# 10XGenomics/thermite

Measured on AMD Instinct MI355X. Metric: aligned reads/sec (91 bp), higher is better.
Workload: dtype i32

## Files before the change

thermite_amd/capi.py:

```python
import ctypes as C
import os

import numpy as np

from .refdata import EXON_DT, REF_DT, SPAN_DT, TX_DT

_HERE = os.path.dirname(os.path.abspath(__file__))
SO_PATH = os.environ.get("THM_LIB") or os.path.join(_HERE, "_build", "libthermite_amd.so")

MEM_DT = np.dtype([("ref_idx", "<u8"), ("query_idx", "<u4"), ("len", "<u4")])
ALN_DT = np.dtype(
    [
        ("ystart", "<u8"),
        ("yend", "<u8"),
        ("ylen", "<u8"),
        ("ops_off", "<u8"),
        ("tx_ystart", "<u8"),
        ("tx_yend", "<u8"),
        ("tx_ylen", "<u8"),
        ("tx_ops_off", "<u8"),
        ("score", "<i4"),
        ("ref_id", "<u4"),
        ("xstart", "<u4"),
        ("xend", "<u4"),
# ... 239 lines not shown
    L.thm_writer_header.restype = i32
    L.thm_writer_header.argtypes = [vp, vp]
    L.thm_writer_trailer.restype = i32
    L.thm_writer_trailer.argtypes = [vp, vp]
    L.thm_writer_format_batch.restype = i32
    L.thm_writer_format_batch.argtypes = [vp, vp, vp, vp]
    L.thm_writer_format_batch_cigars.restype = i32
    L.thm_writer_format_batch_cigars.argtypes = [vp, vp, vp, vp]
    L.thm_batch_upload_reads.restype = i32
    L.thm_batch_upload_reads.argtypes = [vp, vp]
    L.thm_batch_fetch_bam.restype = i32
    L.thm_batch_fetch_bam.argtypes = [vp, u32, vp]
    L.thm_align_batch_bam.restype = i32
    L.thm_align_batch_bam.argtypes = [vp, vp, u32, vp]
    L.thm_writer_wrap_bam.restype = i32
    L.thm_writer_wrap_bam.argtypes = [vp, vp, vp]
    L.thm_align_files.restype = i32
    L.thm_align_files.argtypes = [vp, vp, u32, cp, i32, u64, u32, vp]
    L.thm_align_files_multi.restype = i32
    L.thm_align_files_multi.argtypes = [vp, u32, vp, u32, cp, i32, u64, u32, vp]
    if hasattr(L, "thm_debug_prof_get"):
        L.thm_debug_prof_get.restype = i32
        L.thm_debug_prof_get.argtypes = [vp, vp, i32]
    if hasattr(L, "thm_debug_set_pool_caps"):
        L.thm_debug_set_pool_caps.restype = i32
        L.thm_debug_set_pool_caps.argtypes = [vp, u64, u64, u64, vp]
    if hasattr(L, "thm_debug_set_flags"):
        L.thm_debug_set_flags.restype = i32
        L.thm_debug_set_flags.argtypes = [vp, C.c_uint32]
        L.thm_debug_set_band_clip.restype = i32
        L.thm_debug_set_band_clip.argtypes = [vp, C.c_uint32]
        L.thm_debug_tpr_stats.restype = i32
        L.thm_debug_tpr_stats.argtypes = [vp, vp]
    if hasattr(L, "thm_debug_knobs"):
        L.thm_debug_knobs.restype = i32
        L.thm_debug_knobs.argtypes = [vp, vp]
    if hasattr(L, "thm_debug_calib_gather"):
        L.thm_debug_calib_gather.restype = i32
        L.thm_debug_calib_gather.argtypes = [vp, i32, u64, vp]
    if hasattr(L, "thm_debug_wave_prims"):
        L.thm_debug_wave_prims.restype = i32
        L.thm_debug_wave_prims.argtypes = [vp, vp, vp]
    _lib = L
    return L


def _ptr(a):
    return a.ctypes.data_as(C.c_void_p) if a is not None else None


def _copy(ptr, count, dtype, copy=True):
    if count == 0 or not ptr:
        return np.zeros(0, dtype=dtype)
    nbytes = int(count) * np.dtype(dtype).itemsize
    buf = (C.c_uint8 * nbytes).from_address(ptr)
    a = np.frombuffer(buf, dtype=dtype, count=int(count))
    return a.copy() if copy else a


def _u8(b):
    if isinstance(b, np.ndarray):
        return np.ascontiguousarray(b, np.uint8)
    return np.frombuffer(bytes(b), np.uint8)


def build_suffix_array_gpu(text, wide=False):
# ... 338 lines not shown
                                                  _ptr(hits), len(hits), _ptr(bw), _ptr(xd), max_band_width, C.byref(v)))
        status = (_copy(v.hit_status, v.n_hits, "<i4") if v.hit_status else np.zeros(int(v.n_hits), "<i4"))
        return _copy(v.alns, v.n_hits, ALN_DT), _copy(v.ops, v.n_op_bytes, np.uint8), status

    def counters(self):
        out = np.zeros(N_COUNTERS, "<u8")
        self._chk(lib().thm_counters_get(self.h, _ptr(out)))
        return out

    def reset_counters(self):
        self._chk(lib().thm_counters_reset(self.h))

    def counters_allreduce(self, comm):
        self._chk(lib().thm_counters_allreduce(self.h, comm.h))

    def counters_device_ptr(self):
        return lib().thm_counters_device_ptr(self.h)

    def timings(self):
        out = np.zeros(N_TIMINGS, "<f4")
        self._chk(lib().thm_timings_get(self.h, _ptr(out)))
        return dict(zip(TIMING_NAMES, out.tolist()))

    def debug_prof(self, reset=True):
        out = np.zeros(16, "<u8")
        self._chk(lib().thm_debug_prof_get(self.h, _ptr(out), int(reset)))
        return out

    def debug_set_pool_caps(self, smem_cap=0, cand_cap=0, ops_cap=0):
        n = C.c_uint32()
        self._chk(lib().thm_debug_set_pool_caps(self.h, smem_cap, cand_cap, ops_cap, C.byref(n)))
        return n.value

    def debug_set_flags(self, tpr=None, rounds=0):
        self._chk(lib().thm_debug_set_flags(self.h, (0 if tpr is None else (2 if tpr else 1)) | (int(rounds) << 8)))

    def debug_set_band_clip(self, max_bw=None):
        self._chk(lib().thm_debug_set_band_clip(self.h, 0 if max_bw is None else int(max_bw) + 1))

    def debug_tpr_stats(self):
        out = np.zeros(32, "<u8")
        self._chk(lib().thm_debug_tpr_stats(self.h, _ptr(out)))
        return out

    def debug_knobs(self):
        out = np.zeros(16, "<u4")
        self._chk(lib().thm_debug_knobs(self.h, _ptr(out)))
        return out

    def debug_calib_gather(self, pattern, n_threads):
        b = C.c_uint64()
        self._chk(lib().thm_debug_calib_gather(self.h, pattern, n_threads, C.byref(b)))
        return b.value

    def debug_wave_prims(self, v):
        v = np.ascontiguousarray(v, "<i4")
        out = np.zeros(384, "<i4")
        self._chk(lib().thm_debug_wave_prims(self.h, _ptr(v), _ptr(out)))
        return out.reshape(6, 64)

    def close(self):
        if getattr(self, "h", None):
            lib().thm_aligner_free(self.h)
            self.h = None

    def __del__(self):
        self.close()

# ... 183 lines not shown
```

thermite_amd/csrc/aligner.hip:

```cpp
#include <hip/hip_runtime.h>

#include <algorithm>
#include <cstdarg>
#include <cstdio>
#include <cstdlib>
#include <cstring>
#include <mutex>
#include <string>
#include <type_traits>
#include <vector>

#include "aligner_internal.h"

namespace thm {
const char* global_error_cstr();
}
using namespace thm;

static int swg_blocks_per_cu() {
  static const int v = [] {
    const char* e = getenv("THM_SWG_BPC");
    const int v = e ? atoi(e) : 4;
    return (v >= 1 && v <= 8) ? v : 4;
  }();
// ... 483 lines not shown
  out->n = n;
  out->n_op_bytes = a->h_ops.size();
  out->alns = a->h_lr.data();
  out->ops = a->h_ops.data();
  return THM_OK;
}

int32_t thm_debug_prof_get(thm_aligner* a, uint64_t out[16], int32_t reset) {
  if (!a || !out) return THM_ERR_INVALID_ARG;
  HIPCHK(a, hipSetDevice(a->device));
  uint8_t* p = a->d_counters.as<uint8_t>() + 2 * THM_N_COUNTERS * 8;
  HIPCHK(a, hipMemcpyAsync(out, p, 16 * 8, hipMemcpyDeviceToHost, a->stream));
  if (reset) HIPCHK(a, hipMemsetAsync(p, 0, 16 * 8, a->stream));
  HIPCHK(a, hipStreamSynchronize(a->stream));
  return THM_OK;
}

int32_t thm_debug_set_pool_caps(thm_aligner* a, uint64_t smem_cap, uint64_t cand_cap, uint64_t ops_cap, uint32_t* n_replays) {
  if (!a) return THM_ERR_INVALID_ARG;
  a->dbg_smem_cap = smem_cap;
  a->dbg_cand_cap = cand_cap;
  a->dbg_ops_cap = ops_cap;
  a->smem_cap = a->cand_cap = a->cand_ops_cap = 0;
  if (n_replays) *n_replays = a->n_replays;
  return THM_OK;
}

int32_t thm_debug_set_flags(thm_aligner* a, uint32_t flags) {
  if (!a) return THM_ERR_INVALID_ARG;
  if (flags & 1u) a->use_tpr = false;
  if (flags & 2u) a->use_tpr = true;
  const int r = (int)((flags >> 8) & 15u);
  if (r >= 1 && r <= TPR_MAX_ROUNDS) a->tpr_rounds = r;
  return THM_OK;
}
int32_t thm_debug_set_band_clip(thm_aligner* a, uint32_t max_bw_plus_1) {
  if (!a) return THM_ERR_INVALID_ARG;
  a->dbg_band_clip = max_bw_plus_1;
  return THM_OK;
}
int32_t thm_debug_tpr_stats(thm_aligner* a, uint64_t stats[32]) {
  if (!a || !stats) return THM_ERR_INVALID_ARG;
  memset(stats, 0, 256);
  if (!a->t_ctl.p) return THM_OK;
  HIPCHK(a, hipSetDevice(a->device));
  HIPCHK(a, hipStreamSynchronize(a->stream));
  unsigned long long c[40];
  HIPCHK(a, hipMemcpy(c, a->t_ctl.p, sizeof c, hipMemcpyDeviceToHost));
  for (int k = 0; k < 16; k++) stats[k] = c[TPRC_STATS + k];
  stats[16] = c[TPRC_REC_CUR];
  stats[17] = c[TPRC_Q_CUR];
  for (int k = 0; k < 4; k++) stats[18 + k] = c[TPRC_Q_CUR + 1 + k];
  stats[22] = c[TPRC_N_ACT + a->tpr_rounds + 1];
  return THM_OK;
}
int32_t thm_debug_knobs(thm_aligner* a, uint32_t out[16]) {
  if (!a || !out) return THM_ERR_INVALID_ARG;
  out[0] = seed_fill_mode();
  out[1] = (uint32_t)compact_k();
  out[2] = (uint32_t)hit_gl();
  for (int cpl = 1; cpl <= 4; cpl++)
    for (int wide = 0; wide < 2; wide++) out[3 + 2 * (cpl - 1) + wide] = (uint32_t)extend_waves_per_simd(cpl, wide != 0);
  out[11] = team_div_per_cu();
  out[12] = (uint32_t)swg_blocks_per_cu();
  out[13] = a->use_tpr ? 1u : 0u;
  out[14] = (uint32_t)a->tpr_rounds;
// ... 29 lines not shown
```

thermite_amd/csrc/aligner_internal.h:

```cpp
#ifndef THERMITE_ALIGNER_INTERNAL_H
#define THERMITE_ALIGNER_INTERNAL_H
#include <hip/hip_runtime.h>

#include <cstdarg>
#include <cstdio>
#include <string>
#include <vector>

#include "launch.h"
#include "thermite_internal.h"

struct DBuf {
  void* p = nullptr;
  size_t cap = 0;
  hipError_t ensure(size_t bytes) {
    if (bytes <= cap) return hipSuccess;
    if (p) (void)hipFree(p);
    p = nullptr;
    cap = 0;
    size_t want = bytes + bytes / 4 + 256;
    hipError_t e = hipMalloc(&p, want);
    if (e == hipSuccess) cap = want;
    return e;
  }
// ... 62 lines not shown
  hipStream_t stream3 = nullptr;
  hipEvent_t ev_join3 = nullptr;
  hipStream_t stream4 = nullptr;
  hipEvent_t ev_dpt_fork = nullptr, ev_dpt_join = nullptr;
  hipEvent_t ev_fork = nullptr, ev_join = nullptr;
  thm_align_opts opts;
  std::string err;

  DBuf d_counters, d_queue, d_fault, d_cursors;
  DBuf b0, b1, b2, b3, b4, b5, b6, b7, b8;

  DBuf r_bases, r_offsets, r_san;
  DBuf r_status;
  uint64_t n_reads = 0, n_bases = 0;
  uint32_t max_read_len = 0;
  std::vector<std::pair<uint32_t, uint64_t>> len_hist;
  uint64_t n_over = 0;
  bool uploaded = false;
  DBuf s_smems, s_off, s_cnt, s_hits, s_cand_off, scan_tmp, s_ms_end, s_ms_lo, s_ms_hi, s_work_reads, s_work_long, s_work_cells,
      s_work_counts, s_sel_scratch, s_heavy, s_slow, s_team, s_fill_keys, s_fill_perm, s_fill_hist;
  uint64_t smem_cap = 0;
  DBuf e_heavy, e_rel;
  DBuf e_cands, e_order, e_ops, e_nalns, e_nalns64, e_opbytes, e_aln_off, e_ops_off, e_trace, e_slow, e_recs, e_wcnt;
  DBuf t_memos, t_recs, t_dpops, t_qlist, t_act[2], t_ctl, t_bail, t_queue2, t_trace, t_ttrace, t_hdr, t_sums;
  bool use_tpr = false;
  int tpr_rounds = 8;
  uint64_t n_slow_host = 0;
  uint32_t fast_max_len = 0, slow_max_len = 0;
  uint64_t cand_cap = 0, cand_ops_cap = 0;
  DBuf o_alns, o_ops, o_mems;
  uint64_t out_alns_cap = 0, out_ops_cap = 0;
  uint64_t dbg_smem_cap = 0, dbg_cand_cap = 0, dbg_ops_cap = 0;
  uint32_t dbg_band_clip = 0;
  uint32_t n_replays = 0;
  bool ran = false, synced = false;
  hipEvent_t ev[6] = {nullptr, nullptr, nullptr, nullptr, nullptr, nullptr};
  float timings[THM_N_TIMINGS] = {0};

  HBuf r_off[2], r_alns[2], r_ops[2], r_stat[2];
  int r_cur = 0;
  std::vector<uint64_t> h_off;
  std::vector<thm_aln> h_alns;
  std::vector<uint8_t> h_ops;
  std::vector<thm_mem> h_mems;
  std::vector<thm_swg_aln> h_swg;
  std::vector<thm_lr_aln> h_lr;
  DBuf sh_bases, sh_san, sh_off, sh_hits, sh_read, sh_bw, sh_xd, sh_list, sh_out, sh_status, sh_ops, sh_ctl, sh_trace, sh_slow;
  std::vector<thm_aln> h_hit_alns;
  std::vector<int32_t> h_hit_status;
  std::vector<uint8_t> h_hit_ops;
  DBuf c_sums, c_nwords, c_woff, c_scan_tmp, c_flags, c_dig, c_words, c_in_ops, c_in_off;
  HBuf ch_off[2], ch_alns[2], ch_dig[2], ch_words[2], ch_stat[2];
  int c_cur = 0;
  hipEvent_t ev_cig[4] = {nullptr, nullptr, nullptr, nullptr};
  std::vector<thm_aln_digest> h_cig_dig;
  std::vector<uint32_t> h_cig_words;
  DBuf bn_names, bn_name_off, bn_quals;
  bool reads_named = false, reads_have_quals = false;
  DBuf bt_tx_pool, bt_tx_off, bt_gid_pool, bt_gid_off, bt_gname_pool, bt_gname_off, bt_tx_gene, bt_ref_sq;
  bool bam_tables = false;
  DBuf bm_cnt, bm_first, bm_qn, bm_rec_read, bm_len, bm_off, bm_out, bm_read_off, bm_err, bm_scan_tmp;
  HBuf bh_data[2], bh_off[2], bh_stat[2];
  int b_cur = 0;
  int bam_stage = -1;
  hipEvent_t ev_bam[4] = {nullptr, nullptr, nullptr, nullptr};
};
// ... 28 lines not shown
```

thermite_amd/csrc/kernels_seed.hip:

```cpp
#include <hip/hip_runtime.h>

#include <algorithm>

#include "launch.h"
#include "swg_device.h"

namespace thm {
namespace dev {

__device__ __forceinline__ int base_code(uint8_t c) {
  return c == 'A' ? 0 : c == 'C' ? 1 : c == 'G' ? 2 : c == 'T' ? 3 : -1;
}
__device__ __forceinline__ uint8_t sanitize_base(uint8_t c) {
  if (c >= 'a' && c <= 'z') c = (uint8_t)(c - 32);
  return (c == 'A' || c == 'C' || c == 'G' || c == 'T' || c == 'N') ? c : (uint8_t)0;
}
__device__ __forceinline__ uint64_t load8_global(const uint8_t* p) {
  uint64_t v;
  __builtin_memcpy(&v, p, 8);
  return v;
}
__device__ __forceinline__ uint64_t load8_lds(const uint8_t* base16, int off) {
  const uint64_t* q = (const uint64_t*)(base16 + (off & ~7));
  const unsigned sh = (unsigned)(off & 7) * 8u;
// ... 14 lines not shown
        *less = ((tw >> (8 * idx)) & 0xff) < ((qw >> (8 * idx)) & 0xff);
        return idx;
      }
      return cap;
    }
    o = 8;
  }
  while (o < cap) {
    uint64_t tw[8];
#pragma unroll
    for (int u = 0; u < 8; u++) tw[u] = load8_global(tp + o + 8 * u);
#pragma unroll
    for (int u = 0; u < 8; u++) {
      const int oo = o + 8 * u;
      if (oo < cap) {
        const uint64_t qw = load8_global(q + oo);
        const uint64_t x = tw[u] ^ qw;
        if (x) {
          const int idx = __builtin_ctzll(x) >> 3;
          if (oo + idx < cap) {
            *less = ((tw[u] >> (8 * idx)) & 0xff) < ((qw >> (8 * idx)) & 0xff);
            return oo + idx;
          }
          return cap;
        }
      }
    }
    o += 64;
  }
  return cap;
}

template <class C>
__device__ void ms_search(const DeviceIndexT<C>& ix, const uint8_t* rd, int L, int pos, int k, int& out_d, C& out_lo, C& out_hi) {
  C lo = 0, hi = (C)ix.n;
  int d = 0;
  const int kt = (int)ix.kt;
  if (kt <= k) {
    uint32_t code = 0;
    bool acgt = true;
    const uint64_t w0 = load8_global(rd + pos), w1 = load8_global(rd + pos + 8);
    for (int t = 0; t < kt; t++) {
      const int c = base_code((uint8_t)((t < 8 ? (w0 >> (8 * t)) : (w1 >> (8 * (t - 8)))) & 0xff));
      acgt = acgt && (c >= 0);
      code = (code << 2) | (uint32_t)(c & 3);
    }
    if (acgt) {
      const LutEntryT<C> e = ix.lut[code];
      lo = e.lo;
      hi = e.hi;
      d = kt;
    }
  }
  if (lo < hi && pos + d < L) {
    const int cap = L - (pos + d);
    const uint8_t* q = rd + pos + d;
    bool less;
    const C sz = hi - lo;
    if (sz == 1) {
      d += lcp_cmp<false>(ix.text + ix.sa[lo] + d, q, cap, &less);
    } else if (q[0] != 0) {
      if (sz <= 8) {
        C sav[8];
        uint64_t tw[8];
        int lc[8];
#pragma unroll
        for (int u = 0; u < 8; u++) sav[u] = (lo + u < hi) ? ix.sa[lo + u] : (C)0;
#pragma unroll
        for (int u = 0; u < 8; u++) tw[u] = load8_global(ix.text + sav[u] + d);
        const uint64_t qw = load8_global(q);
        int ms = 0;
#pragma unroll
        for (int u = 0; u < 8; u++) {
          const uint64_t x = tw[u] ^ qw;
          int l = x ? (__builtin_ctzll(x) >> 3) : 8;
          l = min(l, cap);
          if (lo + u >= hi) l = -1;
          lc[u] = l;
        }
#pragma unroll
        for (int u = 0; u < 8; u++) {
          if (lc[u] == 8 && cap > 8) lc[u] = 8 + lcp_cmp<false>(ix.text + sav[u] + d + 8, q + 8, cap - 8, &less);
          ms = max(ms, lc[u]);
        }
// ... 28 lines not shown
          C nlo = a, nhi = a;
          if (l1 >= ms) {
            C x = lo, y = a - 1;
            while (x < y) {
              const C m = x + ((y - x) >> 1);
              if (lcp_cmp<true>(ix.text + ix.sa[m] + d, q, ms, &less) >= ms)
                y = m;
              else
                x = m + 1;
            }
            nlo = x;
          }
          if (l2 >= ms) {
            C x = a + 1, y = hi;
            while (x < y) {
              const C m = x + ((y - x) >> 1);
              if (lcp_cmp<true>(ix.text + ix.sa[m] + d, q, ms, &less) >= ms)
                x = m + 1;
              else
                y = m;
            }
            nhi = x;
          }
          lo = nlo;
          hi = nhi;
          d += ms;
        }
      }
    }
  }
  out_d = (lo < hi) ? d : 0;
  out_lo = lo;
  out_hi = hi;
}

__global__ void sanitize_kernel(const uint8_t* in, uint8_t* out, uint64_t n, uint64_t n_padded) {
  const uint64_t i = ((uint64_t)blockIdx.x * blockDim.x + threadIdx.x) * 16;
  if (i >= n_padded) return;
  uint4 v = make_uint4(0, 0, 0, 0);
  if (i < n) v = *(const uint4*)(in + i);
  uint32_t w[4] = {v.x, v.y, v.z, v.w};
#pragma unroll
  for (int j = 0; j < 4; j++) {
    uint32_t r = 0;
#pragma unroll
    for (int b = 0; b < 4; b++) {
      const uint64_t at = i + (uint64_t)(4 * j + b);
      const uint8_t c = (at < n) ? sanitize_base((uint8_t)(w[j] >> (8 * b))) : (uint8_t)0;
      r |= (uint32_t)c << (8 * b);
    }
    w[j] = r;
  }
  *(uint4*)(out + i) = make_uint4(w[0], w[1], w[2], w[3]);
}

constexpr int PROBE_STRIDE = 8;

__device__ __forceinline__ void block_append(bool flag, unsigned long long value, unsigned long long* list,
                                             unsigned long long* count) {
  __shared__ unsigned w_cnt[4];
  __shared__ unsigned long long b_base;
  const unsigned long long m = __ballot(flag);
  const int lane = lane_id(), wv = (int)(threadIdx.x >> 6);
  if (lane == 0) w_cnt[wv] = (unsigned)__popcll(m);
  __syncthreads();
  if (threadIdx.x == 0) {
    const unsigned total = w_cnt[0] + w_cnt[1] + w_cnt[2] + w_cnt[3];
    b_base = total ? atomicAdd(count, (unsigned long long)total) : 0ull;
  }
  __syncthreads();
  unsigned before = 0;
  for (int w = 0; w < wv; w++) before += w_cnt[w];
  if (flag) list[b_base + before + (unsigned long long)__popcll(m & ((1ull << lane) - 1ull))] = value;
  __syncthreads();
}

template <class C>
__global__ __launch_bounds__(256) void seed_first_kernel(SeedParamsT<C> p) {
  const uint64_t read = (uint64_t)blockIdx.x * 256 + threadIdx.x;
  const int lane = lane_id();
  const bool active = read < p.reads.n_reads;
  const int k = (int)p.min_seed_len;
  int d = 0, L = 0;
  C lo = 0, hi = 0;
  bool too_long = false;
  if (active) {
    const uint64_t r0 = p.reads.offsets[read];
    const uint64_t Lfull = p.reads.offsets[read + 1] - r0;
    too_long = Lfull > MAX_READ_LEN;
    L = too_long ? 0 : (int)Lfull;
    if (too_long) p.read_status[read] = THM_ERR_UNSUPPORTED;
    if (k <= L) ms_search(p.ix, p.reads.bases + r0, L, 0, k, d, lo, hi);
    if (L > 0) {
      const uint64_t item = ms_row(r0, read);
      p.ms_end[item] = (uint16_t)((d >= k) ? d : 0);
      p.ms_lo[item] = lo;
      p.ms_hi[item] = hi;
    }
  }
  const bool covered = active && d >= k && d == L;
  const bool more = active && !covered && L - k + 1 >= 1;
  block_append(more && L <= (int)SHORT_READ_MAX, read, p.work_short, &p.work_counts[0]);
  block_append(more && L > (int)SHORT_READ_MAX, read, p.work_long, &p.work_counts[4]);
  if (active && !covered && !more) {
    p.read_smem_off[read] = 0;
    p.read_smem_cnt[read] = 0;
    p.read_hits[read] = 0;
  }
  const unsigned long long m = __ballot(covered);
  if (m) {
    const int leader = (int)__builtin_ctzll(m);
    unsigned long long base = 0;
    if (lane == leader) base = atomicAdd(p.cursor, (unsigned long long)__popcll(m));
    base = ((unsigned long long)(unsigned)__shfl((int)(base >> 32), leader) << 32) | (unsigned)__shfl((int)(base & 0xffffffffu), leader);
    const bool fits = base + (unsigned long long)__popcll(m) <= p.smem_cap;
    unsigned long long hits = 0;
    if (covered) {
      const unsigned long long slot = base + (unsigned long long)__popcll(m & ((1ull << lane) - 1ull));
      if (fits) {
        SmemT<C> sm;
        sm.lo = lo;
        sm.hi = hi;
        sm.qpos = 0;
        sm.len = (uint16_t)L;
        p.smems[slot] = sm;
      }
      hits = (unsigned long long)(hi - lo);
      p.read_smem_off[read] = slot;
      p.read_smem_cnt[read] = 1u;
      p.read_hits[read] = hits;
    }
    for (int o = 32; o > 0; o >>= 1) hits += __shfl_xor(hits, o);
    if (lane == leader) {
      if (!fits) atomicExch(p.fault, 1);
      atomicAdd(&p.counters[THM_CNT_SMEMS], (unsigned long long)__popcll(m));
      atomicAdd(&p.counters[THM_CNT_HITS], hits);
    }
  }
}

template <class C>
__global__ __launch_bounds__(256) void seed_grid_kernel(SeedParamsT<C> p, const unsigned long long* list,
                                                        const unsigned long long* count, uint32_t G) {
  const uint64_t tid = (uint64_t)blockIdx.x * 256 + threadIdx.x;
  const uint64_t wi = tid / G;
  if (wi >= *count) return;
  const uint64_t read = list[wi];
  const int g = (int)(tid - wi * G);
  const uint64_t r0 = p.reads.offsets[read];
  const int L = (int)(p.reads.offsets[read + 1] - r0);
  const int k = (int)p.min_seed_len;
  const int npos = L - k + 1;
  const int pos = (g + 1 == (int)G) ? npos - 1 : g * PROBE_STRIDE;
  if (pos <= 0 || pos >= npos || (g + 1 != (int)G && pos == npos - 1)) return;
  int d = 0;
  C lo = 0, hi = 0;
  ms_search(p.ix, p.reads.bases + r0, L, pos, k, d, lo, hi);
  const uint64_t item = ms_row(r0, read) + (uint64_t)pos;
  p.ms_end[item] = (uint16_t)((d >= k) ? pos + d : 0);
  p.ms_lo[item] = lo;
  p.ms_hi[item] = hi;
}

template <class C>
__global__ __launch_bounds__(256) void seed_cells_kernel(SeedParamsT<C> p, const unsigned long long* list,
                                                         const unsigned long long* count, uint32_t NC) {
  const uint64_t tid = (uint64_t)blockIdx.x * 256 + threadIdx.x;
  const uint64_t wi = tid / NC;
  bool todo = false;
  uint64_t read = 0;
  int c = 0;
  if (wi < *count) {
    read = list[wi];
    c = (int)(tid - wi * NC);
    const uint64_t r0 = p.reads.offsets[read];
    const int L = (int)(p.reads.offsets[read + 1] - r0);
    const int npos = L - (int)p.min_seed_len + 1;
    const int a = c * PROBE_STRIDE, b = min(a + PROBE_STRIDE, npos - 1);
    if (b - a > 1) {
      const uint64_t item0 = ms_row(r0, read);
      const int ea = p.ms_end[item0 + (uint64_t)a], eb = p.ms_end[item0 + (uint64_t)b];
      if (ea != 0 && ea == eb) {
        for (int q = a + 1; q < b; q++) p.ms_end[item0 + (uint64_t)q] = (uint16_t)ea;
      } else {
        todo = true;
      }
    }
  }
  block_append(todo, (read << 16) | (unsigned long long)c, p.work_cells, &p.work_counts[1]);
}

template <class C>
__device__ __forceinline__ bool fill_item(const SeedParamsT<C>& p, uint64_t tid, uint64_t& read, int& pos, uint64_t& r0, int& L) {
  const int j = (int)(tid % PROBE_STRIDE);
  if (j == 0) return false;
  const unsigned long long w = p.work_cells[tid / PROBE_STRIDE];
  read = w >> 16;
  const int c = (int)(w & 0xffffu);
  r0 = p.reads.offsets[read];
  L = (int)(p.reads.offsets[read + 1] - r0);
  const int npos = L - (int)p.min_seed_len + 1;
  pos = c * PROBE_STRIDE + j;
  return pos < min(c * PROBE_STRIDE + PROBE_STRIDE, npos - 1);
}
template <class C>
__device__ __forceinline__ void fill_probe(const SeedParamsT<C>& p, uint64_t read, int pos, uint64_t r0, int L) {
  const int k = (int)p.min_seed_len;
  int d = 0;
  C lo = 0, hi = 0;
  ms_search(p.ix, p.reads.bases + r0, L, pos, k, d, lo, hi);
  const uint64_t item = ms_row(r0, read) + (uint64_t)pos;
  p.ms_end[item] = (uint16_t)((d >= k) ? pos + d : 0);
  p.ms_lo[item] = lo;
  p.ms_hi[item] = hi;
}

template <class C>
__global__ __launch_bounds__(256) void seed_fill_kernel(SeedParamsT<C> p) {
  const uint64_t total = p.work_counts[1] * PROBE_STRIDE;
  const uint64_t step = (uint64_t)gridDim.x * 256;
  for (uint64_t tid = (uint64_t)blockIdx.x * 256 + threadIdx.x; tid < total; tid += step) {
    uint64_t read, r0;
    int pos, L;
    if (fill_item(p, tid, read, pos, r0, L)) fill_probe(p, read, pos, r0, L);
  }
}

template <class C>
__global__ __launch_bounds__(256) void seed_fill_keys_kernel(SeedParamsT<C> p) {
  const uint64_t total = p.work_counts[1] * PROBE_STRIDE;
  const uint64_t step = (uint64_t)gridDim.x * 256;
  for (uint64_t tid = (uint64_t)blockIdx.x * 256 + threadIdx.x; tid < total; tid += step) {
    uint64_t read, r0;
    int pos, L;
    uint16_t key = 0xFFFF;
    if (fill_item(p, tid, read, pos, r0, L)) {
      const uint64_t w0 = load8_global(p.reads.bases + r0 + pos);
      uint32_t code = 0;
      bool acgt = true;
      for (int t = 0; t < FILL_KEY_BASES; t++) {
        const int c = base_code((uint8_t)((w0 >> (8 * t)) & 0xff));
        acgt = acgt && (c >= 0);
        code = (code << 2) | (uint32_t)(c & 3);
      }
      key = (uint16_t)(acgt ? code : FILL_BUCKETS);
      atomicAdd(&p.fill_hist[key], 1u);
    }
    p.fill_keys[tid] = key;
  }
}
__global__ __launch_bounds__(1024) void seed_fill_scan_kernel(unsigned int* hist) {
  __shared__ unsigned part[1024];
  constexpr unsigned NB = FILL_BUCKETS + 1, PER = (NB + 1023) / 1024;
  const unsigned t = threadIdx.x, b0 = t * PER;
  unsigned sum = 0;
  for (unsigned k = 0; k < PER; k++)
    if (b0 + k < NB) sum += hist[b0 + k];
  part[t] = sum;
  __syncthreads();
  for (unsigned o = 1; o < 1024; o <<= 1) {
    const unsigned v = t >= o ? part[t - o] : 0u;
    __syncthreads();
    part[t] += v;
    __syncthreads();
  }
  unsigned run = part[t] - sum;
  unsigned int* cursor = hist + NB;
  for (unsigned k = 0; k < PER; k++)
    if (b0 + k < NB) {
      cursor[b0 + k] = run;
      run += hist[b0 + k];
    }
  if (t == 1023) hist[2 * NB] = part[1023];
}
template <class C>
__global__ __launch_bounds__(256) void seed_fill_scatter_kernel(SeedParamsT<C> p) {
  const uint64_t total = p.work_counts[1] * PROBE_STRIDE;
  const uint64_t step = (uint64_t)gridDim.x * 256;
  unsigned int* cursor = p.fill_hist + (FILL_BUCKETS + 1);
  for (uint64_t tid = (uint64_t)blockIdx.x * 256 + threadIdx.x; tid < total; tid += step) {
    const uint16_t key = p.fill_keys[tid];
    if (key != 0xFFFF) p.fill_perm[atomicAdd(&cursor[key], 1u)] = (uint32_t)tid;
  }
}
template <class C>
__global__ __launch_bounds__(256) void seed_fill_bucketed_kernel(SeedParamsT<C> p) {
  const uint64_t total = p.fill_hist[2 * (FILL_BUCKETS + 1)];
  const uint64_t step = (uint64_t)gridDim.x * 256;
  for (uint64_t s = (uint64_t)blockIdx.x * 256 + threadIdx.x; s < total; s += step) {
    const uint64_t tid = p.fill_perm[s];
    uint64_t read, r0;
    int pos, L;
    if (fill_item(p, tid, read, pos, r0, L)) fill_probe(p, read, pos, r0, L);
  }
}

template <class C, bool GS>
__global__ __launch_bounds__(256) void seed_select_kernel(SeedParamsT<C> p, const unsigned long long* sel_list,
                                                          const unsigned long long* sel_count, unsigned int* queue, uint32_t lcap) {
  extern __shared__ __attribute__((aligned(16))) uint8_t smem[];
  const int lane = lane_id();
  const int wave = bcast_first((int)(threadIdx.x >> 6));
  const unsigned n_waves = gridDim.x * (blockDim.x >> 6);
  const unsigned wave_global = blockIdx.x * (blockDim.x >> 6) + (unsigned)wave;
  const size_t per_wave = (size_t)lcap * (2 * sizeof(C) + 8);
  uint8_t* base = GS ? p.sel_scratch + (size_t)wave_global * p.sel_scratch_per_wave : smem + (size_t)wave * per_wave;
  C* s_lo = (C*)base;
  C* s_hi = s_lo + lcap;
  uint16_t* a_end = (uint16_t*)(s_hi + lcap);
  uint16_t* s_pos = a_end + lcap;
  uint16_t* s_len = s_pos + lcap;
  uint16_t* s_em = s_len + lcap;
  auto sync = [] {
    if (GS)
      __builtin_amdgcn_fence(__ATOMIC_SEQ_CST, "workgroup");
    else
      __builtin_amdgcn_fence(__ATOMIC_SEQ_CST, "wavefront");
  };

  const int k = (int)p.min_seed_len;
  unsigned long long c_smems = 0, c_hits = 0;
  constexpr unsigned QCHUNK = 8;
  unsigned q_next = 0, q_end = 0;
  const unsigned n_work = (unsigned)uload(sel_count);
  const unsigned n_static_chunks = (unsigned)(((unsigned long long)n_work * 7 / 8) / QCHUNK / n_waves) * n_waves;
  unsigned s_chunk = wave_global;
  unsigned long long pool_off = 0;
// ... 322 lines not shown
}

}

static uint32_t sel_lcap(uint32_t max_read_len) { return (max_read_len + 31u) & ~15u; }
size_t seed_select_scratch_bytes(uint32_t max_read_len) { return (size_t)sel_lcap(max_read_len) * (2 * 8 + 8); }
size_t seed_select_lds_bytes(uint32_t max_read_len) { return 4 * seed_select_scratch_bytes(max_read_len); }

hipError_t launch_sanitize(const uint8_t* in, uint8_t* out, uint64_t n, uint64_t n_padded, hipStream_t s) {
  if (n_padded == 0) return hipSuccess;
  hipLaunchKernelGGL(dev::sanitize_kernel, dim3((unsigned)((n_padded / 16 + 255) / 256 + 1)), dim3(256), 0, s, in, out, n, n_padded);
  return hipGetLastError();
}

template <class C>
static hipError_t launch_seed_t(const SeedParamsT<C>& p, int n_blocks, hipStream_t s) {
  const uint64_t n = p.reads.n_reads;
  if (n == 0) return hipSuccess;
  const uint32_t k = p.min_seed_len;
  auto blocks = [](uint64_t threads) { return dim3((unsigned)((threads + 255) / 256)); };
  auto cells_of = [&](uint32_t max_len) -> uint64_t {
    const uint32_t P = (max_len >= k) ? max_len - k + 1 : 1;
    return (P + dev::PROBE_STRIDE - 1) / dev::PROBE_STRIDE;
  };
  hipError_t e;
  hipLaunchKernelGGL(dev::seed_first_kernel<C>, blocks(n), dim3(256), 0, s, p);
  if ((e = hipGetLastError()) != hipSuccess) return e;
  const uint64_t n_short = n - p.n_long;
  struct Cls {
    uint64_t n;
    uint32_t max_len;
    const unsigned long long* list;
    const unsigned long long* count;
  } cls[2] = {{n_short, p.max_len_short, p.work_short, p.work_counts + 0}, {p.n_long, p.max_len_long, p.work_long, p.work_counts + 4}};
  uint64_t fill_cells = 0;
  for (const Cls& c : cls) {
    if (c.n == 0 || c.max_len < k + 1) continue;
    const uint64_t NC = cells_of(c.max_len), G = NC + 1;
    hipLaunchKernelGGL(dev::seed_grid_kernel<C>, blocks(c.n * G), dim3(256), 0, s, p, c.list, c.count, (uint32_t)G);
    if ((e = hipGetLastError()) != hipSuccess) return e;
    hipLaunchKernelGGL(dev::seed_cells_kernel<C>, blocks(c.n * NC), dim3(256), 0, s, p, c.list, c.count, (uint32_t)NC);
    if ((e = hipGetLastError()) != hipSuccess) return e;
    fill_cells += c.n * NC;
  }
  if (fill_cells) {
    const dim3 worst = blocks(fill_cells * dev::PROBE_STRIDE);
    const dim3 fixed(std::min<unsigned>(worst.x, 256u * 8u * 4u));
    if (p.fill_mode == 2 && fill_cells * dev::PROBE_STRIDE < (1ull << 32)) {
      hipLaunchKernelGGL(dev::seed_fill_keys_kernel<C>, fixed, dim3(256), 0, s, p);
      hipLaunchKernelGGL(dev::seed_fill_scan_kernel, dim3(1), dim3(1024), 0, s, p.fill_hist);
      hipLaunchKernelGGL(dev::seed_fill_scatter_kernel<C>, fixed, dim3(256), 0, s, p);
      hipLaunchKernelGGL(dev::seed_fill_bucketed_kernel<C>, fixed, dim3(256), 0, s, p);
    } else {
      hipLaunchKernelGGL(dev::seed_fill_kernel<C>, p.fill_mode == 1 ? fixed : worst, dim3(256), 0, s, p);
    }
    if ((e = hipGetLastError()) != hipSuccess) return e;
  }
  auto select_waves = [&](const unsigned long long* list, const unsigned long long* count, unsigned int* queue, uint32_t max_len,
                          int nb) -> hipError_t {
    const uint32_t lcap = sel_lcap(max_len);
    const size_t lds = 4 * (size_t)lcap * (2 * sizeof(C) + 8);
    if (lds <= SEED_SELECT_LDS_LIMIT) {
      hipLaunchKernelGGL((dev::seed_select_kernel<C, false>), dim3(nb), dim3(256), lds, s, p, list, count, queue, lcap);
    } else {
      hipLaunchKernelGGL((dev::seed_select_kernel<C, true>), dim3(nb), dim3(256), 0, s, p, list, count, queue, lcap);
    }
    return hipGetLastError();
  };
  if (n_short) {
    unsigned long long* over_list = p.work_cells;
    unsigned long long* over_count = p.work_counts + 3;
    hipLaunchKernelGGL(dev::seed_select_thread_kernel<C>, dim3((unsigned)((n_short + 255) / 256)), dim3(256),
                       (size_t)256 * (2 * sizeof(C) + 4) * dev::SEL_CAP, s, p, over_list, over_count);
    if ((e = hipGetLastError()) != hipSuccess) return e;
    if ((e = select_waves(over_list, over_count, p.queue, p.max_len_short, std::min(n_blocks, 256))) != hipSuccess) return e;
// ... 37 lines not shown
```

thermite_amd/csrc/launch.h:

```cpp
#ifndef THERMITE_LAUNCH_H
#define THERMITE_LAUNCH_H

#include <hip/hip_runtime.h>

#include "thermite_internal.h"

namespace thm {

struct SwgBatchParams {
  const uint8_t* xb;
  const uint64_t* xo;
  const uint8_t* yb;
  const uint64_t* yo;
  const uint32_t* bw;
  const int32_t* xd;
  const uint64_t* ops_off;
  uint8_t* ops;
  thm_swg_aln* out;
  unsigned long long* counters;
  unsigned int* queue;
  int* fault;
  uint64_t n;
  uint32_t x_cap, y_cap;
  uint8_t* scratch;
// ... 25 lines not shown
  uint64_t scratch_per_wave;
  uint32_t max_bw;
};
size_t elr_batch_lds_bytes(const ElrBatchParams& p, int cpl);
size_t elr_batch_scratch_bytes(const ElrBatchParams& p);
hipError_t launch_elr_batch(const ElrBatchParams& p, int cpl, int n_blocks, hipStream_t s);

struct ReadBatch {
  const uint8_t* bases;
  const uint64_t* offsets;
  uint64_t n_reads;
};

constexpr uint32_t MAX_READ_LEN = 65535;
constexpr uint32_t SHORT_READ_MAX = 255;

__host__ __device__ inline uint64_t ms_row(uint64_t base_off, uint64_t r) { return (base_off + 8 * r) & ~7ull; }

template <class C>
struct SeedParamsT {
  DeviceIndexT<C> ix;
  ReadBatch reads;
  uint32_t min_seed_len;
  uint32_t max_len_short;
  uint32_t max_len_long;
  uint64_t n_long;
  uint16_t* ms_end;
  C* ms_lo;
  C* ms_hi;
  unsigned long long* work_short;
  unsigned long long* work_long;
  unsigned long long* work_cells;
  unsigned long long* work_counts;
  SmemT<C>* smems;
  uint64_t smem_cap;
  unsigned long long* cursor;
  uint64_t* read_smem_off;
  uint32_t* read_smem_cnt;
  uint64_t* read_hits;
  int32_t* read_status;
  unsigned long long* counters;
  unsigned int* queue;
  int* fault;
  uint8_t* sel_scratch;
  uint64_t sel_scratch_per_wave;
  uint32_t fill_mode;
  uint16_t* fill_keys;
  uint32_t* fill_perm;
  unsigned int* fill_hist;
};
constexpr int FILL_KEY_BASES = 7;
constexpr unsigned FILL_BUCKETS = 1u << (2 * FILL_KEY_BASES);
size_t seed_select_lds_bytes(uint32_t max_read_len);
size_t seed_select_scratch_bytes(uint32_t max_read_len);
constexpr size_t SEED_SELECT_LDS_LIMIT = 64 * 1024;
hipError_t launch_seed(const SeedParamsT<uint32_t>& p, int n_blocks, hipStream_t s);
hipError_t launch_seed(const SeedParamsT<uint64_t>& p, int n_blocks, hipStream_t s);
hipError_t launch_sanitize(const uint8_t* in, uint8_t* out, uint64_t n, uint64_t n_padded, hipStream_t s);

struct PlanParams {
  const uint64_t* offsets;
  const uint64_t* read_hits;
  uint64_t n_reads;
  uint32_t fast_max_len;
  uint32_t slow_max_len;
  unsigned long long* heavy;
  unsigned long long* slow;
  unsigned long long* team;
  uint32_t team_ok;
  const uint64_t* total_hits;
  uint32_t team_div;
  uint32_t tpr_max_hits;
  unsigned long long* counts;
  int32_t* read_status;
  uint32_t* read_n_alns;
  uint64_t* read_op_bytes;
};
hipError_t launch_plan(const PlanParams& p, hipStream_t s);

template <class C>
struct ReadRecT {
  uint64_t base_off;
  uint64_t smem_off;
// ... 379 lines not shown
```

thermite_amd/csrc/pipeline.hip:

```cpp
#include <hip/hip_runtime.h>

#include <algorithm>
#include <cstring>

#include "aligner_internal.h"

using namespace thm;

uint32_t seed_fill_mode() {
  static const uint32_t v = [] {
    const char* e = getenv("THM_SEED_FILL");
    const int v = e ? atoi(e) : 0;
    return (uint32_t)(v >= 0 && v <= 2 ? v : 0);
  }();
  return v;
}
unsigned team_div_per_cu() {
  static const unsigned v = [] {
    const char* e = getenv("THM_TEAM_DIV_PER_CU");
    const int v = e ? atoi(e) : 0;
    return v > 0 ? (unsigned)v : TEAM_DIV_PER_CU;
  }();
  return v;
}
// ... 40 lines not shown
  HIPCHK(a, a->scan_tmp.ensure(scan_tmp_entries(n + 1) * 8 + 64));
  HIPCHK(a, a->r_status.ensure((n + 1) * 4));
  HIPCHK(a, hipMemsetAsync(a->r_status.p, 0, (n + 1) * 4, s));
  const uint64_t smem_min = a->dbg_smem_cap ? a->dbg_smem_cap : n * 4 + (4u << 20);
  if (a->smem_cap < smem_min) a->smem_cap = smem_min;
  HIPCHK(a, a->s_smems.ensure(a->smem_cap * sizeof(SmemT<C>)));
  if (!a->dbg_smem_cap) a->smem_cap = std::max<uint64_t>(a->smem_cap, a->s_smems.cap / sizeof(SmemT<C>));
  HIPCHK(a, a->r_san.ensure(a->n_bases + 256 + 16));
  HIPCHK(a, hipMemsetAsync(a->r_san.p, 0, 16, s));
  HIPCHK(a, launch_sanitize(a->r_bases.as<uint8_t>(), a->r_san.as<uint8_t>() + 16, a->n_bases, a->n_bases + 128, s));
  uint64_t n_long = 0;
  uint32_t max_short = 0, max_long = 0;
  for (const auto& lc : a->len_hist) {
    if (lc.first <= SHORT_READ_MAX) {
      max_short = std::max(max_short, lc.first);
    } else {
      max_long = std::max(max_long, lc.first);
      n_long += lc.second;
    }
  }
  const uint64_t n_short = n - n_long;
  const uint64_t items = ms_row(a->n_bases, n) + 64;
  HIPCHK(a, a->s_ms_end.ensure(items * 2 + 64));
  HIPCHK(a, a->s_ms_lo.ensure(items * sizeof(C) + 64));
  HIPCHK(a, a->s_ms_hi.ensure(items * sizeof(C) + 64));
  auto cells_of = [&](uint32_t max_len) -> uint64_t {
    const uint32_t P = (max_len >= min_seed_len) ? max_len - min_seed_len + 1 : 1;
    return (P + 7) / 8;
  };
  const uint64_t cells = n_short * cells_of(max_short) + n_long * cells_of(max_long);
  HIPCHK(a, a->s_work_reads.ensure((n + 1) * 8));
  HIPCHK(a, a->s_work_long.ensure((n_long + 1) * 8));
  HIPCHK(a, a->s_work_cells.ensure((std::max(cells, n) + 1) * 8));
  HIPCHK(a, a->s_work_counts.ensure(64));
  HIPCHK(a, hipMemsetAsync(a->s_work_counts.p, 0, 64, s));
  int rc = reset_queue(a);
  if (rc != THM_OK) return rc;
  HIPCHK(a, hipMemsetAsync(a->d_cursors.p, 0, 64, s));
  const int n_blocks = blocks_for(a, n, std::min(seed_select_lds_bytes(std::max(max_short, 1u)), SEED_SELECT_LDS_LIMIT));
  SeedParamsT<C> sp;
  sp.ix = dev_view<C>(a);
  sp.reads.bases = a->r_san.as<uint8_t>() + 16;
  sp.reads.offsets = a->r_offsets.as<uint64_t>();
  sp.reads.n_reads = n;
  sp.min_seed_len = min_seed_len;
  sp.max_len_short = max_short;
  sp.max_len_long = max_long;
  sp.n_long = n_long;
  sp.ms_end = a->s_ms_end.as<uint16_t>();
  sp.ms_lo = a->s_ms_lo.as<C>();
  sp.ms_hi = a->s_ms_hi.as<C>();
  sp.work_short = a->s_work_reads.as<unsigned long long>();
  sp.work_long = a->s_work_long.as<unsigned long long>();
  sp.work_cells = a->s_work_cells.as<unsigned long long>();
  sp.work_counts = a->s_work_counts.as<unsigned long long>();
  sp.smems = a->s_smems.as<SmemT<C>>();
  sp.smem_cap = a->smem_cap;
  sp.cursor = a->d_cursors.as<unsigned long long>();
  sp.read_smem_off = a->s_off.as<uint64_t>();
  sp.read_smem_cnt = a->s_cnt.as<uint32_t>();
  sp.read_hits = a->s_hits.as<uint64_t>();
  sp.read_status = a->r_status.as<int32_t>();
  sp.counters = a->d_counters.as<unsigned long long>();
  sp.queue = a->d_queue.as<unsigned int>();
  sp.fault = a->d_fault.as<int>();
  sp.sel_scratch = nullptr;
  sp.sel_scratch_per_wave = 0;
  const uint32_t fill_mode = seed_fill_mode();
  sp.fill_mode = fill_mode;
  sp.fill_keys = nullptr;
  sp.fill_perm = nullptr;
  sp.fill_hist = nullptr;
  if (fill_mode == 2) {
    const uint64_t slots = (std::max(cells, n) + 1) * 8;
    HIPCHK(a, a->s_fill_keys.ensure(slots * 2));
    HIPCHK(a, a->s_fill_perm.ensure(slots * 4));
    HIPCHK(a, a->s_fill_hist.ensure((2 * (FILL_BUCKETS + 1) + 1) * 4));
    HIPCHK(a, hipMemsetAsync(a->s_fill_hist.p, 0, (2 * (FILL_BUCKETS + 1) + 1) * 4, s));
    sp.fill_keys = a->s_fill_keys.as<uint16_t>();
    sp.fill_perm = a->s_fill_perm.as<uint32_t>();
    sp.fill_hist = a->s_fill_hist.as<unsigned int>();
  }
  if (n_long && seed_select_lds_bytes(max_long) > SEED_SELECT_LDS_LIMIT) {
    const int nb = (int)std::max<uint64_t>(1, std::min<uint64_t>((uint64_t)n_blocks, (n_long + 3) / 4));
    sp.sel_scratch_per_wave = (seed_select_scratch_bytes(max_long) + 255) & ~255ull;
    HIPCHK(a, a->s_sel_scratch.ensure((size_t)nb * 4 * sp.sel_scratch_per_wave + 256));
    sp.sel_scratch = a->s_sel_scratch.as<uint8_t>();
  }
// ... 615 lines not shown
```

Baseline: 86.99 million.

## Infer unique-hit seed extents from neighbors and fuse grid and cell seeding kernels

The seed search now takes a known match-end hint from earlier probes. When the k-mer lookup table already narrows the interval to one suffix and the probe lies inside the known match, it stops early and skips the binary-search extension. For short reads, the grid-probe and cell-classification kernels are fused into one kernel that shares probe results through LDS, which removes a launch and a round trip of ms_end through global memory. Optional seed statistics counters and debug flags are added, and lo/hi are now written only when the end moves past the hint. This changes the store pattern and relies on the inference being exact for unique intervals.

```diff
diff --git a/thermite_amd/capi.py b/thermite_amd/capi.py
--- a/thermite_amd/capi.py
+++ b/thermite_amd/capi.py
@@ -295,6 +295,9 @@
         L.thm_debug_set_band_clip.argtypes = [vp, C.c_uint32]
         L.thm_debug_tpr_stats.restype = i32
         L.thm_debug_tpr_stats.argtypes = [vp, vp]
+    if hasattr(L, "thm_debug_seed_stats"):
+        L.thm_debug_seed_stats.restype = i32
+        L.thm_debug_seed_stats.argtypes = [vp, vp]
     if hasattr(L, "thm_debug_knobs"):
         L.thm_debug_knobs.restype = i32
         L.thm_debug_knobs.argtypes = [vp, vp]
@@ -699,8 +702,16 @@
         self._chk(lib().thm_debug_set_pool_caps(self.h, smem_cap, cand_cap, ops_cap, C.byref(n)))
         return n.value
 
-    def debug_set_flags(self, tpr=None, rounds=0):
-        self._chk(lib().thm_debug_set_flags(self.h, (0 if tpr is None else (2 if tpr else 1)) | (int(rounds) << 8)))
+    def debug_set_flags(self, tpr=None, rounds=0, seed_infer=None, seed_stats=None):
+        word = (0 if tpr is None else (2 if tpr else 1)) | (int(rounds) << 8)
+        word |= 0 if seed_infer is None else (16 if seed_infer else 4)
+        word |= 0 if seed_stats is None else (8 if seed_stats else 32)
+        self._chk(lib().thm_debug_set_flags(self.h, word))
+
+    def debug_seed_stats(self):
+        out = np.zeros(2, "<u8")
+        self._chk(lib().thm_debug_seed_stats(self.h, _ptr(out)))
+        return int(out[0]), int(out[1])
 
     def debug_set_band_clip(self, max_bw=None):
         self._chk(lib().thm_debug_set_band_clip(self.h, 0 if max_bw is None else int(max_bw) + 1))
diff --git a/thermite_amd/csrc/aligner.hip b/thermite_amd/csrc/aligner.hip
--- a/thermite_amd/csrc/aligner.hip
+++ b/thermite_amd/csrc/aligner.hip
@@ -539,6 +539,19 @@
   if (flags & 2u) a->use_tpr = true;
   const int r = (int)((flags >> 8) & 15u);
   if (r >= 1 && r <= TPR_MAX_ROUNDS) a->tpr_rounds = r;
+  if (flags & 4u) a->dbg_seed_noinfer = true;
+  if (flags & 16u) a->dbg_seed_noinfer = false;
+  if (flags & 8u) a->dbg_seed_stats = true;
+  if (flags & 32u) a->dbg_seed_stats = false;
+  return THM_OK;
+}
+int32_t thm_debug_seed_stats(thm_aligner* a, uint64_t stats[2]) {
+  if (!a || !stats) return THM_ERR_INVALID_ARG;
+  stats[0] = stats[1] = 0;
+  if (!a->s_work_counts.p || a->s_work_counts.cap < 128) return THM_OK;
+  HIPCHK(a, hipSetDevice(a->device));
+  HIPCHK(a, hipStreamSynchronize(a->stream));
+  HIPCHK(a, hipMemcpy(stats, a->s_work_counts.as<unsigned long long>() + 8, 16, hipMemcpyDeviceToHost));
   return THM_OK;
 }
 int32_t thm_debug_set_band_clip(thm_aligner* a, uint32_t max_bw_plus_1) {
diff --git a/thermite_amd/csrc/aligner_internal.h b/thermite_amd/csrc/aligner_internal.h
--- a/thermite_amd/csrc/aligner_internal.h
+++ b/thermite_amd/csrc/aligner_internal.h
@@ -118,6 +118,7 @@
   uint64_t out_alns_cap = 0, out_ops_cap = 0;
   uint64_t dbg_smem_cap = 0, dbg_cand_cap = 0, dbg_ops_cap = 0;
   uint32_t dbg_band_clip = 0;
+  bool dbg_seed_noinfer = false, dbg_seed_stats = false;
   uint32_t n_replays = 0;
   bool ran = false, synced = false;
   hipEvent_t ev[6] = {nullptr, nullptr, nullptr, nullptr, nullptr, nullptr};
diff --git a/thermite_amd/csrc/kernels_seed.hip b/thermite_amd/csrc/kernels_seed.hip
--- a/thermite_amd/csrc/kernels_seed.hip
+++ b/thermite_amd/csrc/kernels_seed.hip
@@ -70,7 +70,8 @@
 }
 
 template <class C>
-__device__ void ms_search(const DeviceIndexT<C>& ix, const uint8_t* rd, int L, int pos, int k, int& out_d, C& out_lo, C& out_hi) {
+__device__ bool ms_search(const DeviceIndexT<C>& ix, const uint8_t* rd, int L, int pos, int k, int known_end, int& out_d, C& out_lo,
+                          C& out_hi) {
   C lo = 0, hi = (C)ix.n;
   int d = 0;
   const int kt = (int)ix.kt;
@@ -88,6 +89,12 @@
       lo = e.lo;
       hi = e.hi;
       d = kt;
+      if (known_end != 0 && hi - lo == 1 && pos + kt <= known_end) {
+        out_d = known_end - pos;
+        out_lo = lo;
+        out_hi = hi;
+        return true;
+      }
     }
   }
   if (lo < hi && pos + d < L) {
@@ -182,6 +189,7 @@
   out_d = (lo < hi) ? d : 0;
   out_lo = lo;
   out_hi = hi;
+  return false;
 }
 
 __global__ void sanitize_kernel(const uint8_t* in, uint8_t* out, uint64_t n, uint64_t n_padded) {
@@ -225,12 +233,58 @@
   __syncthreads();
 }
 
+__device__ __forceinline__ unsigned* seed_stats_lds() {
+  __shared__ unsigned s_cnt[2];
+  return s_cnt;
+}
+__device__ __forceinline__ void seed_stats_begin() {
+  unsigned* c = seed_stats_lds();
+  if (threadIdx.x == 0) c[0] = c[1] = 0;
+  __syncthreads();
+}
+__device__ __forceinline__ void seed_stats_note(bool decided) {
+  const unsigned long long here = __ballot(1), dec = __ballot(decided);
+  if (lane_id() == (int)__builtin_ctzll(here)) {
+    unsigned* c = seed_stats_lds();
+    if (dec) atomicAdd(&c[0], (unsigned)__popcll(dec));
+    if (here & ~dec) atomicAdd(&c[1], (unsigned)__popcll(here & ~dec));
+  }
+}
+template <class C>
+__device__ __forceinline__ void seed_stats_end(const SeedParamsT<C>& p) {
+  unsigned* c = seed_stats_lds();
+  __syncthreads();
+  if (threadIdx.x == 0) {
+    if (c[0]) atomicAdd(&p.work_counts[8], (unsigned long long)c[0]);
+    if (c[1]) atomicAdd(&p.work_counts[9], (unsigned long long)c[1]);
+  }
+}
+
+template <class C>
+__device__ __forceinline__ int probe_store(const SeedParamsT<C>& p, const uint8_t* rd, int L, int pos, uint64_t item0, int hint,
+                                           bool& decided) {
+  const int k = (int)p.min_seed_len;
+  int d = 0;
+  C lo = 0, hi = 0;
+  decided = ms_search(p.ix, rd, L, pos, k, hint, d, lo, hi);
+  if (p.flags & SEED_STATS) seed_stats_note(decided);
+  const int e = (d >= k) ? pos + d : 0;
+  const uint64_t item = item0 + (uint64_t)pos;
+  p.ms_end[item] = (uint16_t)e;
+  if (hint == 0 || e > hint) {
+    p.ms_lo[item] = lo;
+    p.ms_hi[item] = hi;
+  }
+  return e;
+}
+
 template <class C>
 __global__ __launch_bounds__(256) void seed_first_kernel(SeedParamsT<C> p) {
   const uint64_t read = (uint64_t)blockIdx.x * 256 + threadIdx.x;
   const int lane = lane_id();
   const bool active = read < p.reads.n_reads;
   const int k = (int)p.min_seed_len;
+  if (p.flags & SEED_STATS) seed_stats_begin();
   int d = 0, L = 0;
   C lo = 0, hi = 0;
   bool too_long = false;
@@ -240,13 +294,17 @@
     too_long = Lfull > MAX_READ_LEN;
     L = too_long ? 0 : (int)Lfull;
     if (too_long) p.read_status[read] = THM_ERR_UNSUPPORTED;
-    if (k <= L) ms_search(p.ix, p.reads.bases + r0, L, 0, k, d, lo, hi);
+    if (k <= L) (void)ms_search(p.ix, p.reads.bases + r0, L, 0, k, 0, d, lo, hi);
     if (L > 0) {
       const uint64_t item = ms_row(r0, read);
       p.ms_end[item] = (uint16_t)((d >= k) ? d : 0);
       p.ms_lo[item] = lo;
       p.ms_hi[item] = hi;
     }
+  }
+  if (p.flags & SEED_STATS) {
+    if (active && k <= L) seed_stats_note(false);
+    seed_stats_end(p);
   }
   const bool covered = active && d >= k && d == L;
   const bool more = active && !covered && L - k + 1 >= 1;
@@ -294,22 +352,68 @@
                                                         const unsigned long long* count, uint32_t G) {
   const uint64_t tid = (uint64_t)blockIdx.x * 256 + threadIdx.x;
   const uint64_t wi = tid / G;
-  if (wi >= *count) return;
-  const uint64_t read = list[wi];
-  const int g = (int)(tid - wi * G);
-  const uint64_t r0 = p.reads.offsets[read];
-  const int L = (int)(p.reads.offsets[read + 1] - r0);
-  const int k = (int)p.min_seed_len;
-  const int npos = L - k + 1;
-  const int pos = (g + 1 == (int)G) ? npos - 1 : g * PROBE_STRIDE;
-  if (pos <= 0 || pos >= npos || (g + 1 != (int)G && pos == npos - 1)) return;
-  int d = 0;
-  C lo = 0, hi = 0;
-  ms_search(p.ix, p.reads.bases + r0, L, pos, k, d, lo, hi);
-  const uint64_t item = ms_row(r0, read) + (uint64_t)pos;
-  p.ms_end[item] = (uint16_t)((d >= k) ? pos + d : 0);
-  p.ms_lo[item] = lo;
-  p.ms_hi[item] = hi;
+  if (p.flags & SEED_STATS) seed_stats_begin();
+  if (wi < *count) {
+    const uint64_t read = list[wi];
+    const int g = (int)(tid - wi * G);
+    const uint64_t r0 = p.reads.offsets[read];
+    const int L = (int)(p.reads.offsets[read + 1] - r0);
+    const int k = (int)p.min_seed_len;
+    const int npos = L - k + 1;
+    const int pos = (g + 1 == (int)G) ? npos - 1 : g * PROBE_STRIDE;
+    if (!(pos <= 0 || pos >= npos || (g + 1 != (int)G && pos == npos - 1))) {
+      const uint64_t item0 = ms_row(r0, read);
+      const int hint = (p.flags & SEED_INFER) ? (int)p.ms_end[item0] : 0;
+      bool decided;
+      (void)probe_store(p, p.reads.bases + r0, L, pos, item0, hint, decided);
+    }
+  }
+  if (p.flags & SEED_STATS) seed_stats_end(p);
+}
+
+template <class C>
+__global__ __launch_bounds__(256) void seed_grid_cells_kernel(SeedParamsT<C> p, const unsigned long long* list,
+                                                              const unsigned long long* count, uint32_t G) {
+  __shared__ uint16_t s_end[256];
+  const unsigned per = 256u / G;
+  const unsigned rl = threadIdx.x / G;
+  const int g = (int)(threadIdx.x - rl * G);
+  const uint64_t wi = (uint64_t)blockIdx.x * per + rl;
+  const bool live = rl < per && wi < *count;
+  if (p.flags & SEED_STATS) seed_stats_begin();
+  uint64_t read = 0, item0 = 0;
+  int npos = 0, e = 0;
+  if (live) {
+    read = list[wi];
+    const uint64_t r0 = p.reads.offsets[read];
+    const int L = (int)(p.reads.offsets[read + 1] - r0);
+    npos = L - (int)p.min_seed_len + 1;
+    item0 = ms_row(r0, read);
+    const int pos = (g + 1 == (int)G) ? npos - 1 : g * PROBE_STRIDE;
+    const int e0 = p.ms_end[item0];
+    if (pos <= 0) {
+      e = e0;
+    } else if (pos < npos && !(g + 1 != (int)G && pos == npos - 1)) {
+      bool decided;
+      e = probe_store(p, p.reads.bases + r0, L, pos, item0, (p.flags & SEED_INFER) ? e0 : 0, decided);
+    }
+  }
+  s_end[threadIdx.x] = (uint16_t)e;
+  __syncthreads();
+  bool todo = false;
+  if (live && g + 1 < (int)G) {
+    const int a = g * PROBE_STRIDE, b = min(a + PROBE_STRIDE, npos - 1);
+    if (b - a > 1) {
+      const int ea = e, eb = s_end[rl * G + (unsigned)(b == npos - 1 ? (int)G - 1 : g + 1)];
+      if (ea != 0 && ea == eb) {
+        for (int q = a + 1; q < b; q++) p.ms_end[item0 + (uint64_t)q] = (uint16_t)ea;
+      } else {
+        todo = true;
+      }
+    }
+  }
+  block_append(todo, (read << 16) | (unsigned long long)g, p.work_cells, &p.work_counts[1]);
+  if (p.flags & SEED_STATS) seed_stats_end(p);
 }
 
 template <class C>
@@ -354,26 +458,41 @@
   return pos < min(c * PROBE_STRIDE + PROBE_STRIDE, npos - 1);
 }
 template <class C>
+__device__ __forceinline__ int fill_hint(const SeedParamsT<C>& p, uint64_t item0, int pos) {
+  const int steps = ((int)p.min_seed_len + PROBE_STRIDE - 1) / PROBE_STRIDE + 1;
+  int a = pos & ~(PROBE_STRIDE - 1);
+  for (int s0 = 0; s0 < steps && a >= 0; s0 += 4, a -= 4 * PROBE_STRIDE) {
+    int e[4];
+#pragma unroll
+    for (int u = 0; u < 4; u++) {
+      const int at = a - u * PROBE_STRIDE;
+      e[u] = (at >= 0 && s0 + u < steps) ? (int)p.ms_end[item0 + (uint64_t)at] : 0;
+    }
+#pragma unroll
+    for (int u = 0; u < 4; u++)
+      if (e[u] != 0) return e[u];
+  }
+  return 0;
+}
+template <class C>
 __device__ __forceinline__ void fill_probe(const SeedParamsT<C>& p, uint64_t read, int pos, uint64_t r0, int L) {
-  const int k = (int)p.min_seed_len;
-  int d = 0;
-  C lo = 0, hi = 0;
-  ms_search(p.ix, p.reads.bases + r0, L, pos, k, d, lo, hi);
-  const uint64_t item = ms_row(r0, read) + (uint64_t)pos;
-  p.ms_end[item] = (uint16_t)((d >= k) ? pos + d : 0);
-  p.ms_lo[item] = lo;
-  p.ms_hi[item] = hi;
+  const uint64_t item0 = ms_row(r0, read);
+  const int hint = (p.flags & SEED_INFER) ? fill_hint(p, item0, pos) : 0;
+  bool decided;
+  (void)probe_store(p, p.reads.bases + r0, L, pos, item0, hint, decided);
 }
 
 template <class C>
 __global__ __launch_bounds__(256) void seed_fill_kernel(SeedParamsT<C> p) {
   const uint64_t total = p.work_counts[1] * PROBE_STRIDE;
   const uint64_t step = (uint64_t)gridDim.x * 256;
+  if (p.flags & SEED_STATS) seed_stats_begin();
   for (uint64_t tid = (uint64_t)blockIdx.x * 256 + threadIdx.x; tid < total; tid += step) {
     uint64_t read, r0;
     int pos, L;
     if (fill_item(p, tid, read, pos, r0, L)) fill_probe(p, read, pos, r0, L);
   }
+  if (p.flags & SEED_STATS) seed_stats_end(p);
 }
 
 template <class C>
@@ -437,12 +556,14 @@
 __global__ __launch_bounds__(256) void seed_fill_bucketed_kernel(SeedParamsT<C> p) {
   const uint64_t total = p.fill_hist[2 * (FILL_BUCKETS + 1)];
   const uint64_t step = (uint64_t)gridDim.x * 256;
+  if (p.flags & SEED_STATS) seed_stats_begin();
   for (uint64_t s = (uint64_t)blockIdx.x * 256 + threadIdx.x; s < total; s += step) {
     const uint64_t tid = p.fill_perm[s];
     uint64_t read, r0;
     int pos, L;
     if (fill_item(p, tid, read, pos, r0, L)) fill_probe(p, read, pos, r0, L);
   }
+  if (p.flags & SEED_STATS) seed_stats_end(p);
 }
 
 template <class C, bool GS>
@@ -831,15 +952,24 @@
     uint32_t max_len;
     const unsigned long long* list;
     const unsigned long long* count;
-  } cls[2] = {{n_short, p.max_len_short, p.work_short, p.work_counts + 0}, {p.n_long, p.max_len_long, p.work_long, p.work_counts + 4}};
+    bool fused;
+  } cls[2] = {{n_short, p.max_len_short, p.work_short, p.work_counts + 0, true},
+              {p.n_long, p.max_len_long, p.work_long, p.work_counts + 4, false}};
   uint64_t fill_cells = 0;
   for (const Cls& c : cls) {
     if (c.n == 0 || c.max_len < k + 1) continue;
     const uint64_t NC = cells_of(c.max_len), G = NC + 1;
-    hipLaunchKernelGGL(dev::seed_grid_kernel<C>, blocks(c.n * G), dim3(256), 0, s, p, c.list, c.count, (uint32_t)G);
-    if ((e = hipGetLastError()) != hipSuccess) return e;
-    hipLaunchKernelGGL(dev::seed_cells_kernel<C>, blocks(c.n * NC), dim3(256), 0, s, p, c.list, c.count, (uint32_t)NC);
-    if ((e = hipGetLastError()) != hipSuccess) return e;
+    if (c.fused && G <= 256) {
+      const uint64_t per = 256 / G;
+      hipLaunchKernelGGL(dev::seed_grid_cells_kernel<C>, dim3((unsigned)((c.n + per - 1) / per)), dim3(256), 0, s, p, c.list, c.count,
+                         (uint32_t)G);
+      if ((e = hipGetLastError()) != hipSuccess) return e;
+    } else {
+      hipLaunchKernelGGL(dev::seed_grid_kernel<C>, blocks(c.n * G), dim3(256), 0, s, p, c.list, c.count, (uint32_t)G);
+      if ((e = hipGetLastError()) != hipSuccess) return e;
+      hipLaunchKernelGGL(dev::seed_cells_kernel<C>, blocks(c.n * NC), dim3(256), 0, s, p, c.list, c.count, (uint32_t)NC);
+      if ((e = hipGetLastError()) != hipSuccess) return e;
+    }
     fill_cells += c.n * NC;
   }
   if (fill_cells) {
diff --git a/thermite_amd/csrc/launch.h b/thermite_amd/csrc/launch.h
--- a/thermite_amd/csrc/launch.h
+++ b/thermite_amd/csrc/launch.h
@@ -81,6 +81,7 @@
   unsigned long long* work_long;
   unsigned long long* work_cells;
   unsigned long long* work_counts;
+  uint32_t flags;
   SmemT<C>* smems;
   uint64_t smem_cap;
   unsigned long long* cursor;
@@ -98,6 +99,7 @@
   uint32_t* fill_perm;
   unsigned int* fill_hist;
 };
+constexpr uint32_t SEED_INFER = 1u, SEED_STATS = 2u;
 constexpr int FILL_KEY_BASES = 7;
 constexpr unsigned FILL_BUCKETS = 1u << (2 * FILL_KEY_BASES);
 size_t seed_select_lds_bytes(uint32_t max_read_len);
diff --git a/thermite_amd/csrc/pipeline.hip b/thermite_amd/csrc/pipeline.hip
--- a/thermite_amd/csrc/pipeline.hip
+++ b/thermite_amd/csrc/pipeline.hip
@@ -96,8 +96,8 @@
   HIPCHK(a, a->s_work_reads.ensure((n + 1) * 8));
   HIPCHK(a, a->s_work_long.ensure((n_long + 1) * 8));
   HIPCHK(a, a->s_work_cells.ensure((std::max(cells, n) + 1) * 8));
-  HIPCHK(a, a->s_work_counts.ensure(64));
-  HIPCHK(a, hipMemsetAsync(a->s_work_counts.p, 0, 64, s));
+  HIPCHK(a, a->s_work_counts.ensure(128));
+  HIPCHK(a, hipMemsetAsync(a->s_work_counts.p, 0, 128, s));
   int rc = reset_queue(a);
   if (rc != THM_OK) return rc;
   HIPCHK(a, hipMemsetAsync(a->d_cursors.p, 0, 64, s));
@@ -118,6 +118,7 @@
   sp.work_long = a->s_work_long.as<unsigned long long>();
   sp.work_cells = a->s_work_cells.as<unsigned long long>();
   sp.work_counts = a->s_work_counts.as<unsigned long long>();
+  sp.flags = (a->dbg_seed_noinfer ? 0u : SEED_INFER) | (a->dbg_seed_stats ? SEED_STATS : 0u);
   sp.smems = a->s_smems.as<SmemT<C>>();
   sp.smem_cap = a->smem_cap;
   sp.cursor = a->d_cursors.as<unsigned long long>();
```

Measured after the change: 88.00 million (median of 6 runs). 1.01x the previous value.
